# ShangHua-Gao/SOD100K

Measured on NVIDIA H100. Metric: images/sec CSNet fwd 224x224, higher is better.
Workload: dtype fp16

## Files before the change

### sod100k_b200/csrc/mix_tc.cuh

```cuda
#pragma once
#include "generic_ops.cuh"
#include "il_block.cuh"

namespace csnet {

constexpr int kTcThreads = 256;
constexpr int kTcWarps = kTcThreads / 32;
constexpr int kTcTH = 8, kTcTW = 32;

struct TcGeom {
  int32_t tiles_x;
  int32_t rows;
  int32_t xs_halves;
  int32_t kc;
  int32_t m16_total;
  const uint16_t* w16[kMaxPaths];
};

__host__ __device__ inline int tc_pad_left(int pad) { return (pad + 3) & ~3; }
__host__ __device__ inline int tc_xw_vec(int pad) { return pad == 0 ? 32 : 64; }
__host__ __device__ inline int tc_xw_exact(int pad) { return (tc_pad_left(pad) + kTcTW + pad + 3) & ~3; }
__host__ __device__ inline int tc_plane_halves(int pad, int rows = 1) {
  int n = (kTcTH * rows + 2 * pad) * tc_xw_vec(pad);
  n = (n + 15) / 16 * 16 + 8;
  return n;
}
__host__ __device__ inline int tc_wrow(int kc) { return kc + 8; }
constexpr int kTcMaxPad = 16;

__device__ __forceinline__ float tc_fetch(const MixPath& P, int64_t plane, int cy, int cx) {
  if (P.up > 1) return bilinear_up(P.src, P.dtype, plane, P.H, P.W, P.up, cy, cx);
  return fetch_pooled(P, plane, cy, cx);
}

template <typename T>
__device__ __forceinline__ float bilinear_up16(const uint16_t* plane, int Hs, int Ws, int up, int oy, int ox) {
  const float inv = 1.0f / (float)up;
  float sy = ((float)oy + 0.5f) * inv - 0.5f, sx = ((float)ox + 0.5f) * inv - 0.5f;
  sy = sy < 0.f ? 0.f : sy;
  sx = sx < 0.f ? 0.f : sx;
  const int y0 = (int)sy, x0 = (int)sx;
  const int y1 = y0 + (y0 < Hs - 1 ? 1 : 0), x1 = x0 + (x0 < Ws - 1 ? 1 : 0);
  const float ly = sy - (float)y0, lx = sx - (float)x0, hy = 1.f - ly, hx = 1.f - lx;
  const uint16_t *r0 = plane + (size_t)y0 * Ws, *r1 = plane + (size_t)y1 * Ws;
  return hy * (hx * Pack<T>::to_f(r0[x0]) + lx * Pack<T>::to_f(r0[x1])) + ly * (hx * Pack<T>::to_f(r1[x0]) + lx * Pack<T>::to_f(r1[x1]));
}

__device__ __forceinline__ void bilinear_up2_pair_f32(const float* plane, int Hs, int Ws, int oy, int ox, float& v0, float& v1) {
  const int i = oy >> 1, j = ox >> 1;
  const int ya = (oy & 1) ? i : (i > 0 ? i - 1 : 0), yb = (oy & 1) ? (i + 1 < Hs ? i + 1 : Hs - 1) : i;
  const float wa = (oy & 1) ? 0.75f : 0.25f, wb = 1.f - wa;
  const int jm = j > 0 ? j - 1 : 0, jp = j + 1 < Ws ? j + 1 : Ws - 1;
  const float *ra = plane + (size_t)ya * Ws, *rb = plane + (size_t)yb * Ws;
  const float am = ra[jm], a0 = ra[j], ap = ra[jp], bm = rb[jm], b0 = rb[j], bp = rb[jp];
  v0 += wa * (0.25f * am + 0.75f * a0) + wb * (0.25f * bm + 0.75f * b0);
  v1 += wa * (0.75f * a0 + 0.25f * ap) + wb * (0.75f * b0 + 0.25f * bp);
}

__device__ __forceinline__ void bilinear_up4n_pair_f32(const float* plane, int Hs, int Ws, int up, int oy, int ox, float& v0, float& v1) {
  const float inv = 1.0f / (float)up;
  float sy = ((float)oy + 0.5f) * inv - 0.5f, sa = ((float)ox + 0.5f) * inv - 0.5f, sb = ((float)(ox + 1) + 0.5f) * inv - 0.5f;
  sy = sy < 0.f ? 0.f : sy;
  sa = sa < 0.f ? 0.f : sa;
  sb = sb < 0.f ? 0.f : sb;
  const int y0 = (int)sy, x0 = (int)sa;
  const int y1 = y0 + (y0 < Hs - 1 ? 1 : 0), x1 = x0 + (x0 < Ws - 1 ? 1 : 0);
  const float ly = sy - (float)y0, hy = 1.f - ly;
  const float la = sa - (float)x0, ha = 1.f - la, lb = sb - (float)x0, hb = 1.f - lb;
  const float *r0 = plane + (size_t)y0 * Ws, *r1 = plane + (size_t)y1 * Ws;
  const float v00 = r0[x0], v01 = r0[x1], v10 = r1[x0], v11 = r1[x1];
  v0 += hy * (ha * v00 + la * v01) + ly * (ha * v10 + la * v11);
  v1 += hy * (hb * v00 + lb * v01) + ly * (hb * v10 + lb * v11);
}

template <typename T>
__device__ __forceinline__ float fetch_pooled16(const MixPath& P, const uint16_t* plane, int y, int x) {
  const int W = P.W, pool = P.pool;
  float m = -INFINITY;
  if (P.pre_avg) {
    const int f = pre_factor(P.pre_avg), fo = (f >> 1) - 1;
    for (int py = 0; py < pool; ++py) {
      const uint16_t* r = plane + (size_t)(f * (y * pool + py) + fo) * W + f * (x * pool) + fo;
      for (int px = 0; px < pool; ++px) {
        const float2 a = Pack<T>::to_f2(*reinterpret_cast<const uint32_t*>(r + f * px));
        const float2 b = Pack<T>::to_f2(*reinterpret_cast<const uint32_t*>(r + W + f * px));
        const float v = (((a.x + a.y) + b.x) + b.y) * 0.25f;
        m = v > m ? v : m;
      }
    }
  } else {
    for (int py = 0; py < pool; ++py) {
      const uint16_t* r = plane + (size_t)(y * pool + py) * W + x * pool;
      for (int px = 0; px < pool; px += 2) {
        const float2 a = Pack<T>::to_f2(*reinterpret_cast<const uint32_t*>(r + px));
        m = fmaxf(m, fmaxf(a.x, a.y));
      }
    }
  }
  return m;
}

template <typename T, int MT, int R = 1>
__global__ void __launch_bounds__(kTcThreads, (MT * R <= 2 ? 3 : 2)) mix_tc_kernel(const __grid_constant__ MixArgs A, const TcGeom G) {
  extern __shared__ __align__(16) uint16_t tc_smem[];
  const int KC = G.kc, WR = tc_wrow(KC);
  uint16_t* Xs = tc_smem;
  uint16_t* Ws = tc_smem + KC * G.xs_halves;
  const int tid = threadIdx.x, lane = tid & 31, warp = tid >> 5;
  const int g = lane >> 2, t = lane & 3;
  const int n = blockIdx.z;
  constexpr int TH = kTcTH * R;
  const int oy0 = (blockIdx.x / G.tiles_x) * TH, ox0 = (blockIdx.x % G.tiles_x) * kTcTW;
  constexpr int M16 = MT * 16;
  const int m_base = blockIdx.y * M16;

  float acc[R][MT][4][4];
#pragma unroll
  for (int r = 0; r < R; ++r)
#pragma unroll
    for (int a = 0; a < MT; ++a)
#pragma unroll
      for (int b = 0; b < 4; ++b)
#pragma unroll
        for (int c = 0; c < 4; ++c) acc[r][a][b][c] = 0.f;

  for (int p0 = 0; p0 < A.n_paths;) {
    const MixPath& P0 = A.p[p0];
    if (P0.ksize == 0) { ++p0; continue; }
    int p1 = p0 + 1, pad = P0.pad;
    while (p1 < A.n_paths) {
      const MixPath& Q = A.p[p1];
      if (Q.ksize == 0 || Q.src != P0.src || Q.c0 != P0.c0 || Q.cin != P0.cin || Q.pre_avg != P0.pre_avg ||
          Q.pool != P0.pool || Q.up != P0.up)
        break;
      pad = Q.pad > pad ? Q.pad : pad;
      ++p1;
    }
    const int cin = P0.cin, srcW = P0.W;
    const int div = pre_factor(P0.pre_avg) * P0.pool;
    const int Hc = P0.up > 1 ? P0.H * P0.up : P0.H / div, Wc = P0.up > 1 ? P0.W * P0.up : P0.W / div;
    const int64_t plane_sz = (int64_t)P0.H * P0.W;
    const bool plain = !P0.pre_avg && P0.pool == 1 && P0.up == 1 && P0.dtype != DT_F32;
    const bool vec = plain && (srcW & 3) == 0;
    const bool pooled16 = P0.dtype != DT_F32 && P0.up == 1 && (P0.pre_avg || P0.pool > 1) && (srcW & 1) == 0 && pre_factor(P0.pre_avg) <= 2;
    const bool up16 = P0.dtype != DT_F32 && P0.up > 1;
    const int XH = TH + 2 * pad, padL = tc_pad_left(pad), PS = tc_plane_halves(pad, R);
    const int XW = vec ? tc_xw_vec(pad) : tc_xw_exact(pad);
    const int64_t src_base = ((int64_t)n * P0.C + P0.c0) * plane_sz;
    for (int c0 = 0; c0 < cin; c0 += KC) {
      const int kc_live = (cin - c0) < KC ? (cin - c0) : KC;
      const int kc8 = (kc_live + 7) & ~7;
      __syncthreads();
      if (vec) {
        const int cs = pad == 0 ? 3 : 4, cmask = (1 << cs) - 1, items = XH << cs;
        const uint16_t* src16 = reinterpret_cast<const uint16_t*>(P0.src) + src_base + (int64_t)c0 * plane_sz;
        for (int ch = warp; ch < kc8; ch += kTcWarps) {
          const bool ch_ok = ch < kc_live;
          const uint16_t* sp = src16 + (int64_t)ch * plane_sz;
          uint16_t* dp = Xs + ch * PS;
          for (int i = lane; i < items; i += 32) {
            const int y = i >> cs, col = i & cmask;
            const int cy = oy0 - pad + y, cx = ox0 - padL + 4 * col;
            const bool ok = ch_ok && cy >= 0 && cy < Hc && cx >= 0 && cx < Wc;
            cp_async8(dp + y * XW + 4 * col, ok ? sp + (int64_t)cy * srcW + cx : sp, ok);
          }
        }
        cp_async_wait_all();
      } else if (up16 && XH * XW <= kTcThreads) {
        const int y = tid / XW, x = tid - y * XW;
        const int cy = oy0 - pad + y, cx = ox0 - padL + x;
        const bool ok = tid < XH * XW && cy >= 0 && cy < Hc && cx >= 0 && cx < Wc;
        const float inv = 1.0f / (float)P0.up;
        float sy = ((float)cy + 0.5f) * inv - 0.5f, sx = ((float)cx + 0.5f) * inv - 0.5f;
        sy = sy < 0.f ? 0.f : sy;
        sx = sx < 0.f ? 0.f : sx;
        const int sy0 = ok ? (int)sy : 0, sx0 = ok ? (int)sx : 0;
        const int sy1 = sy0 + (sy0 < P0.H - 1 ? 1 : 0), sx1 = sx0 + (sx0 < P0.W - 1 ? 1 : 0);
        const float ly = sy - (float)sy0, lx = sx - (float)sx0, hy = 1.f - ly, hx = 1.f - lx;
        const int o00 = sy0 * srcW + sx0, o01 = sy0 * srcW + sx1, o10 = sy1 * srcW + sx0, o11 = sy1 * srcW + sx1;
        const uint16_t* sp = reinterpret_cast<const uint16_t*>(P0.src) + src_base + (int64_t)c0 * plane_sz;
        uint16_t* dp = Xs + y * XW + x;
        if (tid < XH * XW) {
#pragma unroll 4
          for (int ch = 0; ch < kc8; ++ch) {
            float v = 0.f;
            if (ok && ch < kc_live) {
              const uint16_t* pl = sp + (int64_t)ch * plane_sz;
              v = hy * (hx * Pack<T>::to_f(pl[o00]) + lx * Pack<T>::to_f(pl[o01])) + ly * (hx * Pack<T>::to_f(pl[o10]) + lx * Pack<T>::to_f(pl[o11]));
            }
            dp[ch * PS] = (uint16_t)(Pack<T>::from_f2(v, 0.f) & 0xffffu);
          }
        }
      } else {
        for (int ch = warp; ch < kc8; ch += kTcWarps) {
          const bool ch_ok = ch < kc_live;
          const int64_t plane = src_base + (int64_t)(c0 + ch) * plane_sz;
          uint16_t* dp = Xs + ch * PS;
          for (int y0 = 0; y0 < XH; y0 += 4) {
            for (int xb = 0; xb < XW; xb += 32) {
              const int x = xb + lane, cx = ox0 - padL + x;
              const bool col_ok = ch_ok && x < XW && cx >= 0 && cx < Wc;
              float v[4];
#pragma unroll
              for (int q = 0; q < 4; ++q) {
                const int cy = oy0 - pad + y0 + q;
                v[q] = 0.f;
                if (col_ok && y0 + q < XH && cy >= 0 && cy < Hc)
                  v[q] = pooled16 ? fetch_pooled16<T>(P0, reinterpret_cast<const uint16_t*>(P0.src) + plane, cy, cx)
                         : up16 ? bilinear_up16<T>(reinterpret_cast<const uint16_t*>(P0.src) + plane, P0.H, P0.W, P0.up, cy, cx)
                                : tc_fetch(P0, plane, cy, cx);
              }
#pragma unroll
              for (int q = 0; q < 4; ++q)
                if (x < XW && y0 + q < XH) dp[(y0 + q) * XW + x] = (uint16_t)(Pack<T>::from_f2(v[q], 0.f) & 0xffffu);
            }
          }
        }
      }
      for (int p = p0; p < p1; ++p) {
        const MixPath& P = A.p[p];
        const int ksz = P.ksize, kk = ksz * ksz, dil = P.dil;
        if (p > p0) __syncthreads();
        {
          const int vec_row = WR >> 3, per_tap = M16 * vec_row;
          const uint16_t* wsrc = G.w16[p] + ((size_t)(c0 / KC) * kk * G.m16_total + m_base) * WR;
          for (int i = tid; i < kk * per_tap; i += kTcThreads) {
            const int tap = i / per_tap, r = i - tap * per_tap;
            cp_async16(Ws + (size_t)tap * M16 * WR + r * 8, wsrc + (size_t)tap * G.m16_total * WR + r * 8);
          }
          cp_async_wait_all();
        }
        __syncthreads();
        const int off = pad - P.pad, offx = padL - P.pad;
        auto tap = [&](const uint16_t* ra, const uint16_t* rb, const uint16_t* wt) {
          uint32_t af[MT][2];
#pragma unroll
          for (int mt = 0; mt < MT; ++mt) {
            af[mt][0] = *reinterpret_cast<const uint32_t*>(wt + mt * 16 * WR);
            af[mt][1] = *reinterpret_cast<const uint32_t*>(wt + (mt * 16 + 8) * WR);
          }
#pragma unroll
          for (int r = 0; r < R; ++r) {
#pragma unroll
            for (int j = 0; j < 4; ++j) {
              const uint32_t b = __byte_perm((uint32_t)ra[r * 8 * XW + j * 8], (uint32_t)rb[r * 8 * XW + j * 8], 0x5410);
#pragma unroll
              for (int mt = 0; mt < MT; ++mt) Pack<T>::mma(acc[r][mt][j], af[mt], b);
            }
          }
        };
        const int rstep = dil * XW, wstep = M16 * WR;
        for (int ks = 0; ks < kc8; ks += 8) {
          const uint16_t* xa = Xs + (ks + 2 * t) * PS + (warp + off) * XW + g + offx;
          const uint16_t* wt = Ws + g * WR + ks + 2 * t;
          if (ksz == 1 && pad == 0) {
            uint32_t af[MT][2];
#pragma unroll
            for (int mt = 0; mt < MT; ++mt) {
              af[mt][0] = *reinterpret_cast<const uint32_t*>(wt + mt * 16 * WR);
              af[mt][1] = *reinterpret_cast<const uint32_t*>(wt + (mt * 16 + 8) * WR);
            }
#pragma unroll
            for (int r = 0; r < R; ++r) {
              uint32_t bq[4];
              ldmatrix_x4_trans(bq, Xs + (ks + (lane & 7)) * PS + (warp + 8 * r) * XW + (lane >> 3) * 8);
#pragma unroll
              for (int j = 0; j < 4; ++j)
#pragma unroll
                for (int mt = 0; mt < MT; ++mt) Pack<T>::mma(acc[r][mt][j], af[mt], bq[j]);
            }
          } else if (ksz == 1) {
            tap(xa, xa + PS, wt);
          } else {
#pragma unroll 1
            for (int ky = 0; ky < 3; ++ky, xa += rstep) {
              const uint16_t* ra = xa;
#pragma unroll(MT * R <= 1 ? 3 : 1)
              for (int kx = 0; kx < 3; ++kx, ra += dil, wt += wstep) tap(ra, ra + PS, wt);
            }
          }
        }
      }
    }
    p0 = p1;
  }

  uint32_t rmask = 0;
  for (int p = 0; p < A.n_paths; ++p)
    if (A.p[p].ksize == 0) rmask |= 1u << p;
  const int64_t out_plane = (int64_t)A.H * A.W;
  const bool pair_store = A.dtype != DT_F32 && (A.W & 1) == 0;
  const bool proj = A.proj_w != nullptr;
#pragma unroll
  for (int r = 0; r < R; ++r) {
  const int oy = oy0 + warp + 8 * r;
  if (oy >= A.H) break;
  float ps[4][2] = {{0.f, 0.f}, {0.f, 0.f}, {0.f, 0.f}, {0.f, 0.f}};
#pragma unroll
  for (int mt = 0; mt < MT; ++mt) {
#pragma unroll
    for (int h = 0; h < 2; ++h) {
      const int m = m_base + mt * 16 + g + 8 * h;
      if (m >= A.C) continue;
      const float bias = A.bias ? __ldg(A.bias + m) : 0.f;
      const bool has_slope = A.slope != nullptr;
      const float slope_m1 = has_slope ? __ldg(A.slope + m) - 1.f : 0.f;
      const float pw = proj ? __ldg(A.proj_w + m) : 0.f;
      const int64_t orow = ((int64_t)n * A.C + m) * out_plane + (int64_t)oy * A.W;
#pragma unroll
      for (int j = 0; j < 4; ++j) {
        const int ox = ox0 + j * 8 + 2 * t;
        if (ox >= A.W) continue;
        float v0 = acc[r][mt][j][2 * h] + bias, v1 = acc[r][mt][j][2 * h + 1] + bias;
        for (uint32_t mk = rmask; mk; mk &= mk - 1) {
          const MixPath& P = A.p[__ffs(mk) - 1];
          if (m < P.cout0 || m >= P.cout0 + P.cout) continue;
          const int64_t plane = ((int64_t)n * P.C + P.c0 + (m - P.cout0)) * (int64_t)P.H * P.W;
          if (P.up == 2 && P.dtype == DT_F32 && ox + 1 < A.W) {
            bilinear_up2_pair_f32(reinterpret_cast<const float*>(P.src) + plane, P.H, P.W, oy, ox, v0, v1);
          } else if (P.up >= 4 && (P.up & 3) == 0 && P.dtype == DT_F32 && ox + 1 < A.W) {
            bilinear_up4n_pair_f32(reinterpret_cast<const float*>(P.src) + plane, P.H, P.W, P.up, oy, ox, v0, v1);
          } else {
            v0 += bilinear_up(P.src, P.dtype, plane, P.H, P.W, P.up, oy, ox);
            if (ox + 1 < A.W) v1 += bilinear_up(P.src, P.dtype, plane, P.H, P.W, P.up, oy, ox + 1);
          }
        }
        if (has_slope) { v0 = prelu_m1(v0, slope_m1); v1 = prelu_m1(v1, slope_m1); }
        if (proj) {
          ps[j][0] = fmaf(pw, v0, ps[j][0]);
          ps[j][1] = fmaf(pw, v1, ps[j][1]);
        } else if (pair_store) {
          *reinterpret_cast<uint32_t*>(reinterpret_cast<uint16_t*>(A.dst) + orow + ox) = Pack<T>::from_f2(v0, v1);
        } else {
          st_elem(A.dst, A.dtype, orow + ox, v0);
          if (ox + 1 < A.W) st_elem(A.dst, A.dtype, orow + ox + 1, v1);
        }
      }
    }
  }
  if (proj) {
    const float pb = A.proj_b ? __ldg(A.proj_b) : 0.f;
    const int64_t orow = (int64_t)n * out_plane + (int64_t)oy * A.W;
#pragma unroll
    for (int j = 0; j < 4; ++j) {
#pragma unroll
      for (int e = 0; e < 2; ++e) {
        float v = ps[j][e];
        v += __shfl_xor_sync(0xffffffffu, v, 4);
        v += __shfl_xor_sync(0xffffffffu, v, 8);
        v += __shfl_xor_sync(0xffffffffu, v, 16);
        const int ox = ox0 + j * 8 + 2 * t + e;
        if (g == 0 && ox < A.W) st_elem(A.dst, A.dtype, orow + ox, v + pb);
      }
    }
  }
  }
}

}
```

### sod100k_b200/csrc/plan.cu

```cuda
#include <cuda.h>
#include <cuda_runtime.h>

#include <cstdio>
#include <cstdlib>
#include <cstring>
#include <cstdint>
#include <new>
#include <string>
#include <vector>

#include "../../include/csnet_b200.h"
#include "generic_ops.cuh"
#include "il_block.cuh"
#include "il_stream.cuh"
#include "mix_stream.cuh"
#include "ms_direct.cuh"
#include "mix_tc.cuh"
#include "dw_fast.cuh"
#include "image_io.cuh"
#include "resize.cuh"
#include "resize_adj.cuh"

namespace {

// ... 50 lines not shown
}

__global__ void __launch_bounds__(kThreads) dw_generic_kernel(const __grid_constant__ csnet::DwArgs A) {
  const int item = blockIdx.x * kThreads + threadIdx.x;
  const int strips = (A.H + csnet::kDwRows - 1) / csnet::kDwRows;
  if (item >= strips * A.W) return;
  csnet::dw_thread(A, blockIdx.z, blockIdx.y, (item / A.W) * csnet::kDwRows, item % A.W);
}

__global__ void __launch_bounds__(kThreads) gn_stats_kernel(const __grid_constant__ csnet::GnArgs A) {
  const int g = blockIdx.x, n = blockIdx.y, cpg = A.C / A.groups;
  const int64_t base = ((int64_t)n * A.C + (int64_t)g * cpg) * A.HW, cnt = (int64_t)cpg * A.HW;
  __shared__ float sh[2][kThreads / 32];
  __shared__ float mu_s;
  float s = 0.f;
  for (int64_t i = threadIdx.x; i < cnt; i += kThreads) s += csnet::ld_elem(A.src, A.src_dtype, base + i);
  for (int o = 16; o > 0; o >>= 1) s += __shfl_xor_sync(0xffffffffu, s, o);
  if ((threadIdx.x & 31) == 0) sh[0][threadIdx.x >> 5] = s;
  __syncthreads();
  if (threadIdx.x == 0) {
    float t = 0.f;
    for (int i = 0; i < kThreads / 32; ++i) t += sh[0][i];
    mu_s = t / (float)cnt;
  }
  __syncthreads();
  const float mu = mu_s;
  float q = 0.f;
  for (int64_t i = threadIdx.x; i < cnt; i += kThreads) {
    const float d = csnet::ld_elem(A.src, A.src_dtype, base + i) - mu;
    q += d * d;
  }
  for (int o = 16; o > 0; o >>= 1) q += __shfl_xor_sync(0xffffffffu, q, o);
  if ((threadIdx.x & 31) == 0) sh[1][threadIdx.x >> 5] = q;
  __syncthreads();
  if (threadIdx.x == 0) {
    float t = 0.f;
    for (int i = 0; i < kThreads / 32; ++i) t += sh[1][i];
    A.stats[((int64_t)n * A.groups + g) * 2] = mu;
    A.stats[((int64_t)n * A.groups + g) * 2 + 1] = rsqrtf(t / (float)cnt + 1e-5f);
  }
}

__global__ void __launch_bounds__(kThreads) gn_apply_kernel(const __grid_constant__ csnet::GnArgs A) {
  const int c = blockIdx.y, n = blockIdx.z, g = c / (A.C / A.groups);
  const float mu = A.stats[((int64_t)n * A.groups + g) * 2], r = A.stats[((int64_t)n * A.groups + g) * 2 + 1];
  const float ga = A.gamma[c] * r, be = A.beta[c] - mu * ga;
  const bool has_slope = A.slope != nullptr;
  const float sl = has_slope ? A.slope[c] : 1.f;
  const int64_t base = ((int64_t)n * A.C + c) * A.HW;
  for (int i = blockIdx.x * kThreads + threadIdx.x; i < A.HW; i += gridDim.x * kThreads) {
    float v = csnet::ld_elem(A.src, A.src_dtype, base + i) * ga + be;
    if (has_slope) v = v > 0.f ? v : sl * v;
    csnet::st_elem(A.dst, A.dst_dtype, base + i, v);
  }
}

struct PreArgs { double mean[3], std[3]; };
__global__ void __launch_bounds__(kThreads) pre_u8_kernel(const uint8_t* __restrict__ x, float* __restrict__ y, int64_t npix, int64_t hw, const __grid_constant__ PreArgs A) {
  const int64_t i = (int64_t)blockIdx.x * kThreads + threadIdx.x;
  if (i >= npix) return;
  const int64_t n = i / hw, p = i - n * hw;
#pragma unroll
  for (int c = 0; c < 3; ++c) y[(n * 3 + c) * hw + p] = (float)(((double)x[i * 3 + c] / 255.0 - A.mean[c]) / A.std[c]);
}
__global__ void __launch_bounds__(kThreads) post_u8_kernel(const float* __restrict__ z, uint8_t* __restrict__ y, int64_t n) {
  const int64_t i = ((int64_t)blockIdx.x * kThreads + threadIdx.x) * 4;
  if (i >= n) return;
  uchar4 o;
  const float4 v = *reinterpret_cast<const float4*>(z + i);
  o.x = (unsigned char)((1.f / (1.f + expf(-v.x))) * 255.f); o.y = (unsigned char)((1.f / (1.f + expf(-v.y))) * 255.f);
  o.z = (unsigned char)((1.f / (1.f + expf(-v.z))) * 255.f); o.w = (unsigned char)((1.f / (1.f + expf(-v.w))) * 255.f);
  *reinterpret_cast<uchar4*>(y + i) = o;
}

}

struct TcChoice {
  int mt = 0;
  int dtype = 0;
  int xs_halves = 0;
  int rows = 1;
  int kc = 8;
  int kk = 1;
};

enum class Kern : uint8_t { Msd, MixStream, MixTc, Pool2, Upsample, Resample, MixGeneric, Gn, IlStream, IlBlock, DwFast, DwGeneric, Resize };

constexpr int kGraphMaxN = 8;

size_t tc_smem_bytes(const TcChoice& c) {
  return ((size_t)c.kc * c.xs_halves + (size_t)c.kk * c.mt * 16 * (c.kc + 8)) * 2;
}

using IlKernel = void (*)(csnet::IlArgs);
using TcKernel = void (*)(csnet::MixArgs, csnet::TcGeom);

struct OpLaunch {
  Kern kern = Kern::MixGeneric;
  TcChoice tc;
  csnet::MsArgs ms{};
  csnet::IlArgs il{};
  csnet::IlsArgs ils{};
  size_t smem = 0;
  TcKernel tc_fn = nullptr;
  IlKernel il_fn = nullptr;
  uint16_t* w16[CSNET_MAX_PATHS] = {};
};

struct csnet_plan {
  int device = 0;
  int max_batch = 0;
  std::vector<csnet_tensor_desc> tensors;
  std::vector<csnet_op_desc> ops;
  int64_t blob_floats = 0;
  float* blob = nullptr;
  char* arena = nullptr;
  int64_t arena_per_image = 0;
  int n_ext = 0;
  std::vector<OpLaunch> launch;
  struct GraphSlot { cudaGraphExec_t exec = nullptr; void* in = nullptr; void* out = nullptr; size_t in_bytes = 0, out_bytes = 0; };
  std::vector<GraphSlot> graphs;
  cudaStream_t cap_stream = nullptr;
  bool ms_enabled = true;
  int num_sms = 132;
  int ils_force_ns = 0;
  bool ils_enabled = true;
  int ils_min_chunks = 592;
  cudaStream_t s_h2d = nullptr, s_d2h = nullptr;
  void* h_in8[2] = {nullptr, nullptr};
  void* h_out8[2] = {nullptr, nullptr};
  size_t h_in8_bytes = 0, h_out8_bytes = 0;
  csnet_image_geom* h_geom = nullptr;
  int32_t h_geom_n = 0;
  void* h_in[2] = {nullptr, nullptr};
  void* h_out[2] = {nullptr, nullptr};
  size_t h_in_bytes = 0, h_out_bytes = 0;
  cudaEvent_t ev_h2d[2] = {nullptr, nullptr}, ev_comp[2] = {nullptr, nullptr}, ev_d2h[2] = {nullptr, nullptr};
  float* gn_stats = nullptr;
  int gn_groups_max = 0;

  void* tensor_ptr(int t, int N, const void* const* ext) const {
    const csnet_tensor_desc& d = tensors[t];
    if (d.external >= 0) return ext ? const_cast<void*>(ext[d.external]) : nullptr;
    return arena + (int64_t)N * d.arena_offset;
  }
};

namespace {

static inline int mix_channels(const csnet_plan& P, const csnet_op_desc& op) {
  return op.kind == CSNET_OP_MIXPROJ ? (int)op.ext_off[2] : P.tensors[op.dst].C;
}

int validate(const csnet_plan& P) {
  const int nt = (int)P.tensors.size();
  char buf[256];
  for (int t = 0; t < nt; ++t) {
    const csnet_tensor_desc& d = P.tensors[t];
    if (d.C <= 0 || d.H <= 0 || d.W <= 0 || d.dtype < 0 || d.dtype > 2) {
      snprintf(buf, sizeof buf, "tensor %d: bad dims/dtype", t);
      return fail(CSNET_E_INVALID, buf);
    }
    if (d.external < 0 && (d.arena_offset < 0 || d.arena_offset % 256 != 0)) {
      snprintf(buf, sizeof buf, "tensor %d: arena offset must be a non-negative multiple of 256", t);
      return fail(CSNET_E_INVALID, buf);
    }
// ... 347 lines not shown
    const bool k3 = q.ksize == 3 && q.pad == 1 && q.dil == 1, k1 = q.ksize == 1 && q.pad == 0;
    if (A.n_in >= csnet::kMsMaxIn || !(k1 || k3) || (A.n_in > 0 && (int)k3 != A.k3) || q.stride != 1 || q.up != 1 || q.pool != 1 || q.pre_avg ||
        S.dtype != CSNET_F16 || S.H != D.H || S.W != D.W || q.cin > 64)
      return false;
    A.k3 = k3;
    const int i = A.n_in++;
    A.w[i] = P.blob + q.w_off;
    A.cin[i] = q.cin; A.cout0[i] = q.cout0; A.cout[i] = q.cout;
    A.K16[i] = round_up(q.cin, 16); A.S[i] = A.K16[i] + 1;
    if (q.c0 != 0) return false;
  }
  if (A.n_in == 0) return false;
  const int taps = A.k3 ? 9 : 1;
  int wb = 0, smax = 0;
  for (int i = 0; i < A.n_in; ++i) { wb += r128(taps * A.NN * A.K16[i] * 2); smax = A.S[i] > smax ? A.S[i] : smax; }
  auto shape = [&](int rows) {
    csnet::MsArgs T = A;
    T.rows = rows;
    T.nb = (rows * T.G + 7) / 8;
    T.cpi = D.H / rows;
    int off = 0;
    T.tx_bytes = 0;
    for (int i = 0; i < T.n_in; ++i) {
      const int trows = rows + (T.k3 ? 2 : 0);
      T.in_off[i] = off;
      T.copy_bytes[i] = r128(trows * T.G * T.S[i] * 16);
      off += (T.k3 ? 3 : 1) * T.copy_bytes[i];
      T.tx_bytes += trows * T.G * T.S[i] * 16;
    }
    for (int j = 0; j < T.n_rs; ++j) {
      T.r_rows[j] = 0;
      for (int c = 0; c < T.cpi; ++c) {
        const int last = csnet::ms_tap(T.r_H[j], T.r_W[j], T.r_up[j], c * rows + rows - 1, 0).o10 / T.r_W[j];
        const int n = last - csnet::ms_row0(T.r_H[j], T.r_W[j], T.r_up[j], c * rows) + 1;
        T.r_rows[j] = n > T.r_rows[j] ? n : T.r_rows[j];
      }
      T.r_off[j] = off;
      off += r128(T.r_n[j] * T.r_rows[j] * T.r_W[j] * 4);
      T.tx_bytes += T.r_n[j] * T.r_rows[j] * T.r_W[j] * 4;
    }
    T.stage_bytes = off;
    const int slack = (T.nb * 8 - rows * T.G) * smax * 16;
    T.n_stages = (227 * 1024 - (wb + slack + 512 + 1280 + 128)) / T.stage_bytes;
    T.n_stages = T.n_stages > 6 ? 6 : T.n_stages;
    T.off_stage = 0;
    int o = T.n_stages * T.stage_bytes + slack;
    for (int i = 0; i < T.n_in; ++i) { T.off_wb[i] = o; o += r128(taps * T.NN * T.K16[i] * 2); }
    T.off_bar = o; o += 512;
    T.off_tab = o; o += 1280;
    T.smem_bytes = o + 128;
    return T;
  };
  bool found = false;
  for (int rows = 1; rows <= 16 && !found; ++rows) {
    if (D.H % rows) continue;
    const csnet::MsArgs T = shape(rows);
    if (T.nb >= csnet::kMsGroups && T.n_stages >= 3) { A = T; found = true; }
  }
  if (!found) {
    A = shape(csnet::kMsRows);
    if (A.n_stages < 2) A = shape(1);
    if (A.n_stages < 2) return false;
  }
  A.has_slope = op.slope_off >= 0;
  *out = A;
  return true;
}

template <typename T>
IlKernel il_kernel(const csnet::IlArgs& A) {
  if (A.TH == 32) return csnet::il_block_kernel<T, 32, 32>;
  if (A.TH == 28) return csnet::il_block_kernel<T, 28, 32>;
  if (A.TH == 16) return A.TW == 64 ? csnet::il_block_kernel<T, 16, 64> : csnet::il_block_kernel<T, 16, 32>;
  return csnet::il_block_kernel<T, 8, 16>;
}

TcChoice choose_tc(const csnet_plan& P, const csnet_op_desc& op) {
  TcChoice c;
  if (op.kind == CSNET_OP_MIXPROJ) {  }
  else if (op.kind != CSNET_OP_MIX || op.ext_off[23] == 1) return c;
  const csnet_tensor_desc& D = P.tensors[op.dst];
  const int Cm = mix_channels(P, op);
  int dt = D.dtype != CSNET_F32 ? D.dtype : -1, pad = 0, nconv = 0, kk = 1, cin_max = 0;
  for (int p = 0; p < op.n_paths; ++p) {
    const csnet_path_desc& q = op.paths[p];
    if (q.ksize == 0 && (q.pre_avg || q.pool > 1)) return c;
    if (q.ksize == 0) continue;
    ++nconv;
    if (q.stride != 1) return c;
    if (dt < 0 && P.tensors[q.src].dtype != CSNET_F32) dt = P.tensors[q.src].dtype;
    pad = q.pad > pad ? q.pad : pad;
    kk = q.ksize * q.ksize > kk ? q.ksize * q.ksize : kk;
    cin_max = q.cin > cin_max ? q.cin : cin_max;
  }
  if (dt < 0 || nconv == 0 || pad > csnet::kTcMaxPad) return c;
  c.mt = Cm > 80 ? 5 : (Cm + 15) / 16;
  c.dtype = dt;
  c.rows = pad >= 4 ? (c.mt == 1 ? 4 : (c.mt == 2 ? 2 : 1)) : 1;
  c.xs_halves = csnet::tc_plane_halves(pad, c.rows);
  c.kk = kk;
  c.kc = 8;
  for (int kc : {32, 16}) {
    TcChoice t = c;
    t.kc = kc;
    if (kc <= ((cin_max + 7) & ~7) && tc_smem_bytes(t) <= 100 * 1024) { c.kc = kc; break; }
  }
  return c;
}

Kern choose_kernel(const csnet_plan& P, const csnet_op_desc& op, const OpLaunch& R) {
  const csnet_tensor_desc& D = P.tensors[op.dst];
  if (op.kind == CSNET_OP_RESIZE) return Kern::Resize;
  if (is_msd(P, op)) return Kern::Msd;
  if (R.ms.n_in > 0 && (int64_t)P.max_batch * (D.H / csnet::kMsRows) >= (int64_t)2 * P.num_sms) return Kern::MixStream;
  if ((op.kind == CSNET_OP_MIX || op.kind == CSNET_OP_MIXPROJ) && R.tc.mt > 0) return Kern::MixTc;
  if (op.kind == CSNET_OP_MIX && op.n_paths == 1 && op.paths[0].ksize == 0 && op.paths[0].cout0 == 0 && op.paths[0].cout == D.C) {
    const csnet_path_desc& q = op.paths[0];
    const csnet_tensor_desc& Sq = P.tensors[q.src];
    const bool avg2 = q.pre_avg == 1 && q.pool == 1, max2 = q.pre_avg == 0 && q.pool == 2;
    const bool fast = Sq.dtype == D.dtype && D.dtype != CSNET_F32 && D.W % 4 == 0 && op.bias_off < 0 && op.slope_off < 0;
    if (fast && (avg2 || max2) && q.up == 1 && q.c0 == 0) return Kern::Pool2;
    if (fast && q.up > 1 && !q.pre_avg && q.pool == 1) return Kern::Upsample;
    return Kern::Resample;
  }
  if (op.kind == CSNET_OP_MIX) return Kern::MixGeneric;
  if (op.kind == CSNET_OP_GN) return Kern::Gn;
  if (op.kind == CSNET_OP_ILBLOCK)
    return R.ils.ns > 0 && (int64_t)P.max_batch * (D.H / 4) >= (int64_t)P.ils_min_chunks ? Kern::IlStream : Kern::IlBlock;
  const csnet_tensor_desc& Sd = P.tensors[op.paths[0].src];
  return op.ext_off[23] != 1 && Sd.dtype == D.dtype && D.dtype != CSNET_F32 && D.W % 4 == 0 ? Kern::DwFast : Kern::DwGeneric;
}

template <typename T>
TcKernel tc_kernel(const TcChoice& c) {
  if (c.rows == 4) return csnet::mix_tc_kernel<T, 1, 4>;
  if (c.rows == 2) return csnet::mix_tc_kernel<T, 2, 2>;
  switch (c.mt) {
    case 1: return csnet::mix_tc_kernel<T, 1>;
    case 2: return csnet::mix_tc_kernel<T, 2>;
    case 3: return csnet::mix_tc_kernel<T, 3>;
    case 4: return csnet::mix_tc_kernel<T, 4>;
    default: return csnet::mix_tc_kernel<T, 5>;
  }
}

constexpr int kSmemOptIn = 227 * 1024;

const char* const kKernNames[] = {
    "msd_kernel (ms_direct.cuh, FP32 pipe)", "mix_stream_kernel (TMA + wgmma)", "mix_tc_kernel (mma.sync)",
    "pool2 / upsample / resample kernels", "pool2 / upsample / resample kernels", "pool2 / upsample / resample kernels",
    "mix_generic_kernel", "gn kernels", "il_stream_kernel (TMA + wgmma)", "il_block_kernel (mma.sync, tiled)", "dw kernels", "dw kernels",
    "resize_kernel"};
static_assert(sizeof kKernNames / sizeof kKernNames[0] == (size_t)Kern::Resize + 1, "one name per Kern");

int plan_op(csnet_plan& P, size_t i) {
  const csnet_op_desc& op = P.ops[i];
  OpLaunch& R = P.launch[i];
  if (op.kind == CSNET_OP_MIX || op.kind == CSNET_OP_MIXPROJ) {
    R.tc = choose_tc(P, op);
    if (tc_smem_bytes(R.tc) > 200 * 1024) R.tc = TcChoice();
    if (op.kind == CSNET_OP_MIXPROJ && R.tc.mt == 0)
      return fail(CSNET_E_UNSUPPORTED, "MIXPROJ op does not qualify for the tensor-core kernel (16-bit sources, stride 1, pad <= limit)");
    plan_ms(P, op, &R.ms);
  } else if (op.kind == CSNET_OP_ILBLOCK) {
    if (!plan_il(P, op, &R.il)) return fail(CSNET_E_UNSUPPORTED, "ILBLOCK op does not fit shared memory");
    plan_ils(P, op, R.il, &R.ils);
  }
  R.kern = choose_kernel(P, op, R);
  cudaError_t e = cudaSuccess;
  switch (R.kern) {
    case Kern::MixStream:
      e = R.ms.has_proj && R.ms.n_rs > 0
              ? cudaFuncSetAttribute(csnet::mix_stream_kernel<__half, true>, cudaFuncAttributeMaxDynamicSharedMemorySize, kSmemOptIn)
              : cudaFuncSetAttribute(csnet::mix_stream_kernel<__half>, cudaFuncAttributeMaxDynamicSharedMemorySize, kSmemOptIn);
      break;
    case Kern::MixTc: {
      const int C = mix_channels(P, op), slice = R.tc.mt * 16, m16t = (C + slice - 1) / slice * slice, WR = R.tc.kc + 8;
      for (int p = 0; p < op.n_paths; ++p) {
        const csnet_path_desc& q = op.paths[p];
        if (q.ksize == 0) continue;
        const size_t halves = (size_t)((q.cin + R.tc.kc - 1) / R.tc.kc) * q.ksize * q.ksize * m16t * WR;
        e = cudaMalloc(&R.w16[p], halves * 2);
        if (e != cudaSuccess) return fail(CSNET_E_NOMEM, std::string("cudaMalloc(packed weights): ") + cudaGetErrorString(e));
      }
      R.smem = tc_smem_bytes(R.tc);
      R.tc_fn = R.tc.dtype == CSNET_F16 ? tc_kernel<__half>(R.tc) : tc_kernel<__nv_bfloat16>(R.tc);
      e = cudaFuncSetAttribute(R.tc_fn, cudaFuncAttributeMaxDynamicSharedMemorySize, kSmemOptIn);
      break;
    }
    case Kern::IlStream: {
      const bool stem = R.ils.Ci > 0;
      e = cudaFuncSetAttribute(stem ? csnet::il_stream_kernel<__half, true> : csnet::il_stream_kernel<__half, false>,
                               cudaFuncAttributeMaxDynamicSharedMemorySize, kSmemOptIn);
      if (e == cudaSuccess && !stem)
        e = cudaFuncSetAttribute(csnet::il_stream_kernel<__half, false>, cudaFuncAttributePreferredSharedMemoryCarveout, 100);
      break;
    }
    case Kern::IlBlock:
      R.smem = il_smem_of(R.il);
      R.il_fn = P.tensors[op.dst].dtype == CSNET_F16 ? il_kernel<__half>(R.il) : il_kernel<__nv_bfloat16>(R.il);
      e = cudaFuncSetAttribute(R.il_fn, cudaFuncAttributeMaxDynamicSharedMemorySize, kSmemOptIn);
      break;
    default:
      break;
  }
  if (e != cudaSuccess)
    return fail(CSNET_E_CUDA, std::string("cudaFuncSetAttribute(") + kKernNames[(int)R.kern] + "): " + cudaGetErrorString(e));
  return CSNET_OK;
}

}

namespace csnet {
void train_set_error(const char* msg);
}

extern "C" {
// ... 110 lines not shown
        for (int tap = 0; tap < kk; ++tap)
          for (int co = 0; co < q.cout; ++co) {
            const float v = w[((size_t)ci * kk + tap) * q.cout + co];
            uint16_t bits;
            if (tc.dtype == CSNET_F16) { __half hv = __float2half_rn(v); memcpy(&bits, &hv, 2); }
            else { __nv_bfloat16 hv = __float2bfloat16_rn(v); memcpy(&bits, &hv, 2); }
            h[(((size_t)(ci / tc.kc) * kk + tap) * m16t + q.cout0 + co) * WR + ci % tc.kc] = bits;
          }
      CU_CHECK(cudaMemcpyAsync(R.w16[p], h.data(), h.size() * 2, cudaMemcpyHostToDevice, (cudaStream_t)stream));
      keep.push_back(std::move(h));
    }
  }
  CU_CHECK(cudaStreamSynchronize((cudaStream_t)stream));
  return CSNET_OK;
}

static int check_run_args(csnet_plan* P, int32_t N, const void* const* ext_ptrs, int32_t n_ext) {
  if (!P) return fail(CSNET_E_INVALID, "null plan");
  if (N <= 0 || N > P->max_batch) return fail(CSNET_E_INVALID, "batch size outside [1, max_batch]");
  if (n_ext < P->n_ext || (P->n_ext > 0 && !ext_ptrs)) return fail(CSNET_E_INVALID, "missing external tensor pointers");
  for (int i = 0; i < P->n_ext; ++i)
    if (!ext_ptrs[i]) return fail(CSNET_E_INVALID, "null external tensor pointer");
  return CSNET_OK;
}

static int launch_op(csnet_plan* P, size_t i, int32_t N, const void* const* ext_ptrs, cudaStream_t stream) {
  const csnet_op_desc& op = P->ops[i];
  const csnet_tensor_desc& D = P->tensors[op.dst];
  const OpLaunch& R = P->launch[i];
  switch (R.kern) {
    case Kern::Msd:
      for (int p = 0; p < op.n_paths; ++p) {
        const csnet_path_desc& q = op.paths[p];
        csnet::MsdArgs A{};
        A.src = reinterpret_cast<const uint16_t*>(P->tensor_ptr(q.src, N, ext_ptrs));
        A.dst = reinterpret_cast<uint16_t*>(P->tensor_ptr(op.dst, N, ext_ptrs));
        A.w = P->blob + q.w_off;
        A.bias = op.bias_off >= 0 ? P->blob + op.bias_off : nullptr;
        A.slope = op.slope_off >= 0 ? P->blob + op.slope_off : nullptr;
        A.N = N; A.Cin = q.cin; A.H = D.H; A.W = D.W; A.Ctot = D.C; A.cout0 = q.cout0; A.cout = q.cout;
        csnet::msd_launch<__half>(q.dil, A, stream);
      }
      break;
    case Kern::MixStream: {
      csnet::MsArgs A = R.ms;
      A.N = N;
      A.total_chunks = N * A.cpi;
      A.dst = P->tensor_ptr(op.dst, N, ext_ptrs);
      CUtensorMap maps[csnet::kMsMaxIn], rmaps[csnet::kMsMaxRs];
      memset(maps, 0, sizeof maps);
      for (int p = 0, in = 0, rs = 0; p < op.n_paths; ++p) {
        const csnet_path_desc& q = op.paths[p];
        const csnet_tensor_desc& S = P->tensors[q.src];
        if (q.ksize == 0) {
          if (!encode_image_map(&rmaps[rs], P->tensor_ptr(q.src, N, ext_ptrs), N, S.C, S.H, S.W, S.W, A.r_rows[rs], A.r_n[rs]))
            return fail(CSNET_E_CUDA, "cuTensorMapEncodeTiled failed (streaming MIX)");
          ++rs;
          continue;
        }
        if (!encode_group_map(&maps[in], P->tensor_ptr(q.src, N, ext_ptrs), N, S.C, S.H, S.W, A.S[in], A.G, A.rows + (A.k3 ? 2 : 0)))
          return fail(CSNET_E_CUDA, "cuTensorMapEncodeTiled failed (streaming MIX)");
        ++in;
      }
      for (int k = A.n_in; k < csnet::kMsMaxIn; ++k) maps[k] = maps[0];
      for (int k = A.n_rs; k < csnet::kMsMaxRs; ++k) rmaps[k] = maps[0];
      int grid = A.total_chunks / 2;
      grid = grid < 1 ? 1 : (grid > P->num_sms ? P->num_sms : grid);
      if (A.has_proj && A.n_rs > 0)
        csnet::mix_stream_kernel<__half, true><<<grid, csnet::kMsThreads, A.smem_bytes, stream>>>(A, maps[0], maps[1], maps[2], rmaps[0], rmaps[1]);
      else
        csnet::mix_stream_kernel<__half><<<grid, csnet::kMsThreads, A.smem_bytes, stream>>>(A, maps[0], maps[1], maps[2], rmaps[0], rmaps[1]);
      break;
    }
    case Kern::MixTc: {
      csnet::MixArgs A = make_mix(*P, op, N, ext_ptrs);
      const TcChoice& tc = R.tc;
      const int Cm = A.C;
      csnet::TcGeom G{};
      G.tiles_x = (D.W + csnet::kTcTW - 1) / csnet::kTcTW; G.xs_halves = tc.xs_halves; G.kc = tc.kc; G.rows = tc.rows;
      const int th = csnet::kTcTH * tc.rows;
      G.m16_total = (Cm + tc.mt * 16 - 1) / (tc.mt * 16) * (tc.mt * 16);
      for (int p = 0; p < op.n_paths; ++p) G.w16[p] = R.w16[p];
      dim3 grid(G.tiles_x * ((D.H + th - 1) / th), (Cm + tc.mt * 16 - 1) / (tc.mt * 16), N);
      R.tc_fn<<<grid, csnet::kTcThreads, R.smem, stream>>>(A, G);
      break;
    }
    case Kern::Pool2: {
      csnet::MixArgs A = make_mix(*P, op, N, ext_ptrs);
      const bool max2 = op.paths[0].pool == 2;
      const dim3 grid((D.H * (D.W / 4) + 255) / 256, D.C, N);
      if (D.dtype == CSNET_F16) csnet::pool2_fast_kernel<__half><<<grid, 256, 0, stream>>>(A, max2);
      else csnet::pool2_fast_kernel<__nv_bfloat16><<<grid, 256, 0, stream>>>(A, max2);
      break;
    }
    case Kern::Upsample: {
      csnet::MixArgs A = make_mix(*P, op, N, ext_ptrs);
      const dim3 grid((D.H * (D.W / 4) + 255) / 256, D.C, N);
      if (D.dtype == CSNET_F16) csnet::upsample_fast_kernel<__half><<<grid, 256, 0, stream>>>(A);
      else csnet::upsample_fast_kernel<__nv_bfloat16><<<grid, 256, 0, stream>>>(A);
      break;
    }
    case Kern::Resample:
      csnet::resample_fast_kernel<<<dim3((D.H * D.W + 255) / 256, D.C, N), 256, 0, stream>>>(make_mix(*P, op, N, ext_ptrs));
      break;
    case Kern::MixGeneric: {
      dim3 grid((D.H * D.W + kThreads - 1) / kThreads, (D.C + csnet::kMixCT - 1) / csnet::kMixCT, N);
      mix_generic_kernel<<<grid, kThreads, 0, stream>>>(make_mix(*P, op, N, ext_ptrs));
      break;
    }
    case Kern::Gn: {
      const csnet_tensor_desc& S = P->tensors[op.paths[0].src];
      csnet::GnArgs A{};
      A.src = P->tensor_ptr(op.paths[0].src, N, ext_ptrs);
      A.dst = P->tensor_ptr(op.dst, N, ext_ptrs);
      A.gamma = P->blob + op.ext_off[0];
      A.beta = P->blob + op.ext_off[1];
      A.slope = op.slope_off >= 0 ? P->blob + op.slope_off : nullptr;
      A.stats = P->gn_stats;
      A.src_dtype = S.dtype; A.dst_dtype = D.dtype; A.C = D.C; A.HW = D.H * D.W; A.groups = op.paths[0].up;
      gn_stats_kernel<<<dim3(A.groups, N), kThreads, 0, stream>>>(A);
      const int bx = (A.HW + kThreads * 4 - 1) / (kThreads * 4);
      gn_apply_kernel<<<dim3(bx < 1 ? 1 : bx, D.C, N), kThreads, 0, stream>>>(A);
      break;
    }
    case Kern::IlStream: {
      csnet::IlsArgs A = R.ils;
      A.yh = P->tensor_ptr(op.dst, N, ext_ptrs);
      A.yl = op.dst2 >= 0 ? P->tensor_ptr(op.dst2, N, ext_ptrs) : nullptr;
      A.N = N;
      A.total_chunks = N * A.ns * A.cpi;
      CUtensorMap tmH, tmL;
      const bool stem = A.Ci > 0;
      if (stem) {
        if (!encode_image_map(&tmL, P->tensor_ptr(op.paths[0].src, N, ext_ptrs), N, A.Ci, A.H, A.W, A.BW, 4, A.Ci))
          return fail(CSNET_E_CUDA, "cuTensorMapEncodeTiled failed (streaming ILBlock, image)");
        tmH = tmL;
      } else if (!encode_group_map(&tmH, P->tensor_ptr(op.paths[0].src, N, ext_ptrs), N, A.Chi, A.H, A.W, A.SH, A.GR, 4) ||
                 !encode_group_map(&tmL, P->tensor_ptr(op.paths[1].src, N, ext_ptrs), N, A.Cli, A.H / 2, A.W / 2, A.SL, A.GLR, 2))
        return fail(CSNET_E_CUDA, "cuTensorMapEncodeTiled failed (streaming ILBlock)");
      int grid = A.total_chunks / 4;
      grid = grid < 1 ? 1 : (grid > P->num_sms ? P->num_sms : grid);
      if (stem) csnet::il_stream_kernel<__half, true><<<grid, A.dw_warps * 32, A.smem_bytes, stream>>>(A, tmH, tmL);
      else csnet::il_stream_kernel<__half, false><<<grid, A.dw_warps * 32, A.smem_bytes, stream>>>(A, tmH, tmL);
      break;
    }
    case Kern::IlBlock: {
      csnet::IlArgs A = R.il;
      A.xh = P->tensor_ptr(op.paths[0].src, N, ext_ptrs);
      if (!A.first) A.xl = P->tensor_ptr(op.paths[1].src, N, ext_ptrs);
      A.yh = P->tensor_ptr(op.dst, N, ext_ptrs);
      if (op.dst2 >= 0) A.yl = P->tensor_ptr(op.dst2, N, ext_ptrs);
      const int tiles_y = (A.H + A.TH - 1) / A.TH;
      dim3 grid(A.tiles_x * tiles_y, 1, N);
      R.il_fn<<<grid, csnet::kIlThreads, R.smem, stream>>>(A);
      break;
    }
    case Kern::DwFast:
    case Kern::DwGeneric: {
      const csnet_path_desc& q = op.paths[0];
      const csnet_tensor_desc& S = P->tensors[q.src];
      csnet::DwArgs A{};
      A.src = P->tensor_ptr(q.src, N, ext_ptrs);
      A.dst = P->tensor_ptr(op.dst, N, ext_ptrs);
      A.w = P->blob + q.w_off;
      A.bias = op.bias_off >= 0 ? P->blob + op.bias_off : nullptr;
      A.slope = op.slope_off >= 0 ? P->blob + op.slope_off : nullptr;
// ... 485 lines not shown
```

Before: 18470.

## Add flat batch-pixel tiling for small-resolution 1x1 tensor-core mix convs

For 1x1 convolutions on small feature maps (at most 1024 pixels), the tensor-core mix kernel now treats the batch and spatial dimensions as one flat pixel index. Each 256-pixel block can then span several images instead of leaving most of an 8x32 tile idle at 7x7 or 14x14 resolutions. Loads use 16-byte cp.async when possible, and the epilogue walks image, row and column per pixel pair. It also adds a 4-byte cp.async path for even-width unvectorised inputs, and drops the wait after the vector load, which may be a correctness risk if no later wait exists.

```diff
diff --git a/sod100k_b200/csrc/mix_tc.cuh b/sod100k_b200/csrc/mix_tc.cuh
--- a/sod100k_b200/csrc/mix_tc.cuh
+++ b/sod100k_b200/csrc/mix_tc.cuh
@@ -7,6 +7,7 @@
 constexpr int kTcThreads = 256;
 constexpr int kTcWarps = kTcThreads / 32;
 constexpr int kTcTH = 8, kTcTW = 32;
+constexpr int kTcFlatMaxPixels = 32 * 32;
 
 struct TcGeom {
   int32_t tiles_x;
@@ -14,6 +15,7 @@
   int32_t xs_halves;
   int32_t kc;
   int32_t m16_total;
+  int32_t flat_total;
   const uint16_t* w16[kMaxPaths];
 };
 
@@ -100,8 +102,16 @@
   return m;
 }
 
-template <typename T, int MT, int R = 1>
+__device__ __forceinline__ void cp_async4(void* dst, const void* src, bool valid) {
+  asm volatile("cp.async.ca.shared.global [%0], [%1], 4, %2;\n" ::"r"(smem_u32(dst)), "l"(src), "r"(valid ? 4 : 0) : "memory");
+}
+__device__ __forceinline__ void cp_async16z(void* dst, const void* src, bool valid) {
+  asm volatile("cp.async.cg.shared.global [%0], [%1], 16, %2;\n" ::"r"(smem_u32(dst)), "l"(src), "r"(valid ? 16 : 0) : "memory");
+}
+
+template <typename T, int MT, int R = 1, bool FLAT = false>
 __global__ void __launch_bounds__(kTcThreads, (MT * R <= 2 ? 3 : 2)) mix_tc_kernel(const __grid_constant__ MixArgs A, const TcGeom G) {
+  static_assert(!FLAT || R == 1, "the FLAT form has one 32-pixel run per warp");
   extern __shared__ __align__(16) uint16_t tc_smem[];
   const int KC = G.kc, WR = tc_wrow(KC);
   uint16_t* Xs = tc_smem;
@@ -110,9 +120,14 @@
   const int g = lane >> 2, t = lane & 3;
   const int n = blockIdx.z;
   constexpr int TH = kTcTH * R;
-  const int oy0 = (blockIdx.x / G.tiles_x) * TH, ox0 = (blockIdx.x % G.tiles_x) * kTcTW;
+  const int oy0 = FLAT ? 0 : (blockIdx.x / G.tiles_x) * TH, ox0 = FLAT ? 0 : (blockIdx.x % G.tiles_x) * kTcTW;
   constexpr int M16 = MT * 16;
   const int m_base = blockIdx.y * M16;
+  const int hw = A.H * A.W;
+  const int pix0 = blockIdx.x * (kTcTH * kTcTW);
+  const bool flat16 = (hw & 7) == 0;
+  const int f_col = flat16 ? (tid & 31) : (tid & 63), f_q = pix0 + (flat16 ? 8 : 4) * f_col;
+  const int f_img = FLAT ? f_q / hw : 0, f_p = f_q - f_img * hw;
 
   float acc[R][MT][4][4];
 #pragma unroll
@@ -151,7 +166,22 @@
       const int kc_live = (cin - c0) < KC ? (cin - c0) : KC;
       const int kc8 = (kc_live + 7) & ~7;
       __syncthreads();
-      if (vec) {
+      if (FLAT) {
+        const uint16_t* src16 = reinterpret_cast<const uint16_t*>(P0.src);
+        const int64_t img_base = ((int64_t)f_img * P0.C + P0.c0 + c0) * plane_sz + f_p;
+        const bool q_ok = f_q < G.flat_total;
+        if (flat16) {
+          for (int ch = tid >> 5; ch < kc8; ch += kTcThreads / 32) {
+            const bool ok = q_ok && ch < kc_live;
+            cp_async16z(Xs + ch * PS + 8 * f_col, ok ? src16 + img_base + (int64_t)ch * plane_sz : src16, ok);
+          }
+        } else {
+          for (int ch = tid >> 6; ch < kc8; ch += kTcThreads / 64) {
+            const bool ok = q_ok && ch < kc_live;
+            cp_async8(Xs + ch * PS + 4 * f_col, ok ? src16 + img_base + (int64_t)ch * plane_sz : src16, ok);
+          }
+        }
+      } else if (vec) {
         const int cs = pad == 0 ? 3 : 4, cmask = (1 << cs) - 1, items = XH << cs;
         const uint16_t* src16 = reinterpret_cast<const uint16_t*>(P0.src) + src_base + (int64_t)c0 * plane_sz;
         for (int ch = warp; ch < kc8; ch += kTcWarps) {
@@ -165,7 +195,21 @@
             cp_async8(dp + y * XW + 4 * col, ok ? sp + (int64_t)cy * srcW + cx : sp, ok);
           }
         }
-        cp_async_wait_all();
+      } else if (plain && (srcW & 1) == 0) {
+        const uint16_t* src16 = reinterpret_cast<const uint16_t*>(P0.src) + src_base + (int64_t)c0 * plane_sz;
+        for (int ch = warp; ch < kc8; ch += kTcWarps) {
+          const bool ch_ok = ch < kc_live;
+          const uint16_t* sp = src16 + (int64_t)ch * plane_sz;
+          uint16_t* dp = Xs + ch * PS;
+          for (int y = 0; y < XH; ++y) {
+            const int cy = oy0 - pad + y;
+            for (int col = lane; 2 * col < XW; col += 32) {
+              const int cx = ox0 - padL + 2 * col;
+              const bool ok = ch_ok && cy >= 0 && cy < Hc && cx >= 0 && cx < Wc;
+              cp_async4(dp + y * XW + 2 * col, ok ? sp + (int64_t)cy * srcW + cx : sp, ok);
+            }
+          }
+        }
       } else if (up16 && XH * XW <= kTcThreads) {
         const int y = tid / XW, x = tid - y * XW;
         const int cy = oy0 - pad + y, cx = ox0 - padL + x;
@@ -293,8 +337,24 @@
   const bool proj = A.proj_w != nullptr;
 #pragma unroll
   for (int r = 0; r < R; ++r) {
-  const int oy = oy0 + warp + 8 * r;
-  if (oy >= A.H) break;
+  if (!FLAT && oy0 + warp + 8 * r >= A.H) break;
+  int n_0 = n, oy_0 = oy0 + warp + 8 * r, ox_0 = ox0 + 2 * t;
+  const int q_0 = pix0 + warp * kTcTW + 2 * t;
+  if (FLAT) {
+    n_0 = q_0 / hw;
+    const int p = q_0 - n_0 * hw;
+    oy_0 = p / A.W;
+    ox_0 = p - oy_0 * A.W;
+  }
+  auto next_pair = [&](int& img, int& oy, int& ox) {
+    ox += 8;
+    if (FLAT)
+      while (ox >= A.W) {
+        ox -= A.W;
+        if (++oy == A.H) { oy = 0; ++img; }
+      }
+  };
+  auto live = [&](int j, int ox) { return FLAT ? q_0 + 8 * j < G.flat_total : ox < A.W; };
   float ps[4][2] = {{0.f, 0.f}, {0.f, 0.f}, {0.f, 0.f}, {0.f, 0.f}};
 #pragma unroll
   for (int mt = 0; mt < MT; ++mt) {
@@ -306,25 +366,36 @@
       const bool has_slope = A.slope != nullptr;
       const float slope_m1 = has_slope ? __ldg(A.slope + m) - 1.f : 0.f;
       const float pw = proj ? __ldg(A.proj_w + m) : 0.f;
-      const int64_t orow = ((int64_t)n * A.C + m) * out_plane + (int64_t)oy * A.W;
+      float v[4][2];
+#pragma unroll
+      for (int j = 0; j < 4; ++j) { v[j][0] = acc[r][mt][j][2 * h] + bias; v[j][1] = acc[r][mt][j][2 * h + 1] + bias; }
+      for (uint32_t mk = rmask; mk; mk &= mk - 1) {
+        const MixPath& P = A.p[__ffs(mk) - 1];
+        if (m < P.cout0 || m >= P.cout0 + P.cout) continue;
+        const bool up2 = P.up == 2 && P.dtype == DT_F32, up4n = P.up >= 4 && (P.up & 3) == 0 && P.dtype == DT_F32;
+        int img = n_0, oy = oy_0, ox = ox_0;
+#pragma unroll
+        for (int j = 0; j < 4; ++j) {
+          if (j > 0) next_pair(img, oy, ox);
+          if (!live(j, ox)) continue;
+          const int64_t plane = ((int64_t)img * P.C + P.c0 + (m - P.cout0)) * (int64_t)P.H * P.W;
+          if (up2 && ox + 1 < A.W) {
+            bilinear_up2_pair_f32(reinterpret_cast<const float*>(P.src) + plane, P.H, P.W, oy, ox, v[j][0], v[j][1]);
+          } else if (up4n && ox + 1 < A.W) {
+            bilinear_up4n_pair_f32(reinterpret_cast<const float*>(P.src) + plane, P.H, P.W, P.up, oy, ox, v[j][0], v[j][1]);
+          } else {
+            v[j][0] += bilinear_up(P.src, P.dtype, plane, P.H, P.W, P.up, oy, ox);
+            if (ox + 1 < A.W) v[j][1] += bilinear_up(P.src, P.dtype, plane, P.H, P.W, P.up, oy, ox + 1);
+          }
+        }
+      }
+      int img = n_0, oy = oy_0, ox = ox_0;
 #pragma unroll
       for (int j = 0; j < 4; ++j) {
-        const int ox = ox0 + j * 8 + 2 * t;
-        if (ox >= A.W) continue;
-        float v0 = acc[r][mt][j][2 * h] + bias, v1 = acc[r][mt][j][2 * h + 1] + bias;
-        for (uint32_t mk = rmask; mk; mk &= mk - 1) {
-          const MixPath& P = A.p[__ffs(mk) - 1];
-          if (m < P.cout0 || m >= P.cout0 + P.cout) continue;
-          const int64_t plane = ((int64_t)n * P.C + P.c0 + (m - P.cout0)) * (int64_t)P.H * P.W;
-          if (P.up == 2 && P.dtype == DT_F32 && ox + 1 < A.W) {
-            bilinear_up2_pair_f32(reinterpret_cast<const float*>(P.src) + plane, P.H, P.W, oy, ox, v0, v1);
-          } else if (P.up >= 4 && (P.up & 3) == 0 && P.dtype == DT_F32 && ox + 1 < A.W) {
-            bilinear_up4n_pair_f32(reinterpret_cast<const float*>(P.src) + plane, P.H, P.W, P.up, oy, ox, v0, v1);
-          } else {
-            v0 += bilinear_up(P.src, P.dtype, plane, P.H, P.W, P.up, oy, ox);
-            if (ox + 1 < A.W) v1 += bilinear_up(P.src, P.dtype, plane, P.H, P.W, P.up, oy, ox + 1);
-          }
-        }
+        if (j > 0) next_pair(img, oy, ox);
+        if (!live(j, ox)) continue;
+        const int64_t orow = ((int64_t)img * A.C + m) * out_plane + (int64_t)oy * A.W;
+        float v0 = v[j][0], v1 = v[j][1];
         if (has_slope) { v0 = prelu_m1(v0, slope_m1); v1 = prelu_m1(v1, slope_m1); }
         if (proj) {
           ps[j][0] = fmaf(pw, v0, ps[j][0]);
@@ -340,21 +411,23 @@
   }
   if (proj) {
     const float pb = A.proj_b ? __ldg(A.proj_b) : 0.f;
-    const int64_t orow = (int64_t)n * out_plane + (int64_t)oy * A.W;
+    int img = n_0, oy = oy_0, ox = ox_0;
 #pragma unroll
     for (int j = 0; j < 4; ++j) {
+      if (j > 0) next_pair(img, oy, ox);
+      const bool st = g == 0 && live(j, ox);
+      const int64_t orow = (int64_t)img * out_plane + (int64_t)oy * A.W;
 #pragma unroll
       for (int e = 0; e < 2; ++e) {
         float v = ps[j][e];
         v += __shfl_xor_sync(0xffffffffu, v, 4);
         v += __shfl_xor_sync(0xffffffffu, v, 8);
         v += __shfl_xor_sync(0xffffffffu, v, 16);
-        const int ox = ox0 + j * 8 + 2 * t + e;
-        if (g == 0 && ox < A.W) st_elem(A.dst, A.dtype, orow + ox, v + pb);
-      }
-    }
-  }
-  }
-}
-
-}
+        if (st && ox + e < A.W) st_elem(A.dst, A.dtype, orow + ox + e, v + pb);
+      }
+    }
+  }
+  }
+}
+
+}
diff --git a/sod100k_b200/csrc/plan.cu b/sod100k_b200/csrc/plan.cu
--- a/sod100k_b200/csrc/plan.cu
+++ b/sod100k_b200/csrc/plan.cu
@@ -156,6 +156,7 @@
   int rows = 1;
   int kc = 8;
   int kk = 1;
+  bool flat = false;
 };
 
 enum class Kern : uint8_t { Msd, MixStream, MixTc, Pool2, Upsample, Resample, MixGeneric, Gn, IlStream, IlBlock, DwFast, DwGeneric, Resize };
@@ -669,11 +670,14 @@
   const csnet_tensor_desc& D = P.tensors[op.dst];
   const int Cm = mix_channels(P, op);
   int dt = D.dtype != CSNET_F32 ? D.dtype : -1, pad = 0, nconv = 0, kk = 1, cin_max = 0;
+  bool flat = (int64_t)D.H * D.W <= csnet::kTcFlatMaxPixels && (D.H * D.W) % 4 == 0 && D.W % 2 == 0;
   for (int p = 0; p < op.n_paths; ++p) {
     const csnet_path_desc& q = op.paths[p];
     if (q.ksize == 0 && (q.pre_avg || q.pool > 1)) return c;
     if (q.ksize == 0) continue;
     ++nconv;
+    const csnet_tensor_desc& S = P.tensors[q.src];
+    flat = flat && q.ksize == 1 && q.pad == 0 && !q.pre_avg && q.pool == 1 && q.up == 1 && S.dtype != CSNET_F32 && S.H == D.H && S.W == D.W;
     if (q.stride != 1) return c;
     if (dt < 0 && P.tensors[q.src].dtype != CSNET_F32) dt = P.tensors[q.src].dtype;
     pad = q.pad > pad ? q.pad : pad;
@@ -683,6 +687,7 @@
   if (dt < 0 || nconv == 0 || pad > csnet::kTcMaxPad) return c;
   c.mt = Cm > 80 ? 5 : (Cm + 15) / 16;
   c.dtype = dt;
+  c.flat = flat;
   c.rows = pad >= 4 ? (c.mt == 1 ? 4 : (c.mt == 2 ? 2 : 1)) : 1;
   c.xs_halves = csnet::tc_plane_halves(pad, c.rows);
   c.kk = kk;
@@ -720,6 +725,15 @@
 
 template <typename T>
 TcKernel tc_kernel(const TcChoice& c) {
+  if (c.flat) {
+    switch (c.mt) {
+      case 1: return csnet::mix_tc_kernel<T, 1, 1, true>;
+      case 2: return csnet::mix_tc_kernel<T, 2, 1, true>;
+      case 3: return csnet::mix_tc_kernel<T, 3, 1, true>;
+      case 4: return csnet::mix_tc_kernel<T, 4, 1, true>;
+      default: return csnet::mix_tc_kernel<T, 5, 1, true>;
+    }
+  }
   if (c.rows == 4) return csnet::mix_tc_kernel<T, 1, 4>;
   if (c.rows == 2) return csnet::mix_tc_kernel<T, 2, 2>;
   switch (c.mt) {
@@ -996,6 +1010,10 @@
       G.m16_total = (Cm + tc.mt * 16 - 1) / (tc.mt * 16) * (tc.mt * 16);
       for (int p = 0; p < op.n_paths; ++p) G.w16[p] = R.w16[p];
       dim3 grid(G.tiles_x * ((D.H + th - 1) / th), (Cm + tc.mt * 16 - 1) / (tc.mt * 16), N);
+      if (tc.flat) {
+        G.flat_total = N * D.H * D.W;
+        grid = dim3((G.flat_total + csnet::kTcTH * csnet::kTcTW - 1) / (csnet::kTcTH * csnet::kTcTW), grid.y, 1);
+      }
       R.tc_fn<<<grid, csnet::kTcThreads, R.smem, stream>>>(A, G);
       break;
     }
```

Measured after the change: 18980, median of 6. 1.03x the previous value.
